# sontung/pyrenderer

Hardware: AMD Instinct MI355X
Metric: Msamples/sec Cornell box 512²×64spp at 1/2/4/8 GPU; per-pixel L2 vs CPU (higher is better)
Workload: dtype f32; 1 GPU; Cornell box (Lambertian) 512x512, 64 spp, depth 8; triangles=36, spheres=0, global_batch=16777216, parallelism=tiles1, collective=False, tile_scheme=latin, frames_in_flight=1, frames_per_launch=16, tile=64, bvh_depth=8, bvh_nodes=18

## Files before the change

### pyrenderer_amd/csrc/prt_capi.cpp

```cpp
#include <dlfcn.h>
#include <hip/hip_runtime.h>
#include <rccl/rccl.h>

#include <algorithm>
#include <cmath>
#include <cstdlib>
#include <cstring>
#include <map>
#include <memory>
#include <mutex>
#include <new>
#include <string>
#include <vector>

#include "../../include/prt.h"
#include "prt_internal.h"
#include "prt_kernels.h"

namespace {

thread_local std::string g_err;

int fail(int code, const std::string& msg) {
    g_err = msg;
// ... 3 lines not shown
#define HIP_TRY(expr)                                                                         \
    do {                                                                                      \
        hipError_t e_ = (expr);                                                               \
        if (e_ != hipSuccess) return fail(PRT_ERR_HIP, std::string(#expr) + ": " + hipGetErrorString(e_)); \
    } while (0)

float bits_f(int32_t v) { float f; std::memcpy(&f, &v, 4); return f; }

struct F3 { float x, y, z; };
F3 f3_norm(F3 a) {
    float l = std::sqrt(a.x * a.x + a.y * a.y + a.z * a.z);
    return F3{a.x / l, a.y / l, a.z / l};
}
F3 f3_cross(F3 a, F3 b) { return F3{a.y * b.z - a.z * b.y, a.z * b.x - a.x * b.z, a.x * b.y - a.y * b.x}; }
void frame_rows(F3 n, float* out12) {
    F3 v = f3_norm(n);
    F3 r1, r2, r3;
    if (v.y == 1.0f) {
        r1 = F3{1, 0, 0}; r2 = F3{0, 0, 1}; r3 = F3{0, 1, 0};
    } else if (v.y == -1.0f) {
        r1 = F3{1, 0, 0}; r2 = F3{0, 0, 1}; r3 = F3{0, -1, 0};
    } else {
        F3 x = f3_norm(f3_cross(v, F3{0.0f, 1.0f, 0.0f}));
        F3 z = f3_norm(f3_cross(x, v));
        r1 = x; r2 = z; r3 = v;
    }
    const F3 rows[3] = {r1, r2, r3};
    for (int k = 0; k < 3; ++k) {
        out12[4 * k] = rows[k].x; out12[4 * k + 1] = rows[k].y; out12[4 * k + 2] = rows[k].z; out12[4 * k + 3] = 0.0f;
    }
}

constexpr int kStatWords = 192;

struct DevBuf {
    void* p = nullptr;
    size_t bytes = 0;
    DevBuf() = default;
    DevBuf(const DevBuf&) = delete;
    DevBuf& operator=(const DevBuf&) = delete;
    ~DevBuf() { release(); }
    hipError_t ensure(size_t want) {
        if (want <= bytes) return hipSuccess;
        if (p) (void)hipFree(p);
        p = nullptr; bytes = 0;
        hipError_t e = hipMalloc(&p, want);
        if (e == hipSuccess) bytes = want;
        return e;
    }
    void release() { if (p) (void)hipFree(p); p = nullptr; bytes = 0; }
};

struct RenderCtx {
    hipStream_t stream = nullptr;
    DevBuf tiles, buf, rays, rays_o, work, acc, spill;
    std::vector<uint32_t> tile_host;
    uint64_t last_use = 0;
};
constexpr size_t kMaxCtx = 8;

struct Scene {
    int device = 0;
    int64_t n_tri = 0;
    int64_t n_nodes = 0;
    int32_t depth = 0;
    int n_light = 0;
    int n_mat = 0;
    int cus = 0;
    int blocks_per_cu = 0;
    int occ[2 * (prt::kVarLast + 1)] = {0};
    int n_lt = 0;
    int64_t n_tri_f4 = 0;
    float direct_rgb[3] = {0.9f, 0.85f, 0.7f};
    DevBuf nodes4q;
    int64_t n_node4q_f4 = 0;
    DevBuf nodes4, tris, tri_nm, tri_frame, mats, light_v, light_off, sph, sph_mat;
    int64_t n_node4_f4 = 0;
    int32_t depth4 = 0;
    int stack4 = 0;
    int need4 = 0;
    int leaf_break = -1;
    int leaf_exit = -1;
    int resume_min = 32;
    uint32_t guard_trips = 1u << 20;
    int spill_lds = 16;
    std::string wave_clock_path;
    int64_t n_sph = 0;
    bool plain = false;
    bool shade_fast = false;
    DevBuf work, stats;
    hipStream_t stream = nullptr;
    std::vector<std::unique_ptr<RenderCtx>> ctx;
    uint64_t use_clock = 0;
    std::vector<hipEvent_t> ev;
    int ev_used = 0;
    size_t chunk_bytes = (size_t)16 << 30;
    size_t device_bytes = 0;
    DevBuf frame, gather, gather_xy;
    std::vector<uint32_t> gather_xy_host;
    DevBuf scatter_xy;
    std::vector<uint32_t> scatter_xy_host;
    hipEvent_t scatter_ev = nullptr;
};

struct DeviceGuard {
    int prev = -1;
    explicit DeviceGuard(int dev) { (void)hipGetDevice(&prev); (void)hipSetDevice(dev); }
    ~DeviceGuard() { if (prev >= 0) (void)hipSetDevice(prev); }
};

int upload(DevBuf& b, const void* host, size_t bytes, size_t* total) {
    HIP_TRY(b.ensure(std::max<size_t>(bytes, 16)));
    if (bytes) HIP_TRY(hipMemcpy(b.p, host, bytes, hipMemcpyHostToDevice));
    *total += b.bytes;
    return PRT_OK;
}

void destroy_scene(Scene* s) {
    if (!s) return;
    DeviceGuard g(s->device);
    for (DevBuf* b : {&s->nodes4q, &s->nodes4, &s->tris, &s->tri_nm, &s->tri_frame, &s->mats, &s->light_v,
                      &s->light_off, &s->sph, &s->sph_mat, &s->work, &s->stats, &s->frame, &s->gather,
                      &s->gather_xy, &s->scatter_xy})
        b->release();
    if (!s->ctx.empty()) (void)hipDeviceSynchronize();
    for (auto& c : s->ctx)
        for (DevBuf* b : {&c->tiles, &c->buf, &c->rays, &c->rays_o, &c->work, &c->acc, &c->spill})
            b->release();
    for (hipEvent_t e : s->ev) (void)hipEventDestroy(e);
    if (s->scatter_ev) (void)hipEventDestroy(s->scatter_ev);
    if (s->stream) (void)hipStreamDestroy(s->stream);
    delete s;
}

int check_render_args(Scene* s, const float* cam, int W, int H, int tw, int th, const int32_t* tile_ids,
                      int n_tiles, int spp, int depth) {
    if (!s) return fail(PRT_ERR_ARG, "scene is NULL");
    if (!cam) return fail(PRT_ERR_ARG, "cam is NULL");
    if (W < 2 || H < 2) return fail(PRT_ERR_ARG, "W and H must be >= 2 (u = (x + r) / (W - 1))");
    if (tw < 1 || th < 1 || (tw & (tw - 1)) || (th & (th - 1)) || (int64_t)tw * th < 64 || (int64_t)tw * th > (1 << 20))
        return fail(PRT_ERR_ARG, "tile width/height must be powers of two with 64 <= tw*th <= 2^20");
    if (W > 65535 || H > 65535) return fail(PRT_ERR_ARG, "frame larger than 65535 pixels per side");
    if (n_tiles < 0 || (n_tiles > 0 && !tile_ids)) return fail(PRT_ERR_ARG, "bad tile list");
    if (spp < 0 || depth < 0) return fail(PRT_ERR_ARG, "spp and depth must be >= 0");
    int tiles_x = (W + tw - 1) / tw, tiles_y = (H + th - 1) / th;
    for (int i = 0; i < n_tiles; ++i)
        if (tile_ids[i] < 0 || tile_ids[i] >= tiles_x * tiles_y)
            return fail(PRT_ERR_ARG, "tile id out of range: " + std::to_string(tile_ids[i]));
    if ((int64_t)n_tiles * tw * th >= ((int64_t)1 << 31)) return fail(PRT_ERR_ARG, "too many pixels in one call");
    return PRT_OK;
}

constexpr size_t kFaultOffset = 32;

int take_fault_at(const DevBuf& work) {
    int f = 0;
    if (!work.p) return 0;
    if (hipMemcpy(&f, (char*)work.p + kFaultOffset, sizeof(int), hipMemcpyDeviceToHost) != hipSuccess) return -1;
    if (f != 0 && hipMemset((char*)work.p + kFaultOffset, 0, sizeof(int)) != hipSuccess) return -1;
    return f;
}
int take_fault(Scene* s) { return take_fault_at(s->work); }
int take_render_faults(Scene* s) {
    int any = 0;
    for (auto& c : s->ctx)
        if (int f = take_fault_at(c->work)) any = any ? any : f;
    return any;
}

RenderCtx* ctx_for(Scene* s, hipStream_t stream) {
    ++s->use_clock;
    for (auto& c : s->ctx)
        if (c->stream == stream) { c->last_use = s->use_clock; return c.get(); }
    if (s->ctx.size() >= kMaxCtx) {
        auto it = std::min_element(s->ctx.begin(), s->ctx.end(),
                                   [](const std::unique_ptr<RenderCtx>& a, const std::unique_ptr<RenderCtx>& b) {
                                       return a->last_use < b->last_use;
                                   });
        if (hipDeviceSynchronize() != hipSuccess) return nullptr;
        (*it)->stream = stream;
        (*it)->last_use = s->use_clock;
        return it->get();
    }
    auto c = std::unique_ptr<RenderCtx>(new (std::nothrow) RenderCtx());
    if (!c) return nullptr;
    if (c->work.ensure(64) != hipSuccess) return nullptr;
    if (hipMemset(c->work.p, 0, 64) != hipSuccess) return nullptr;
    c->stream = stream;
    c->last_use = s->use_clock;
    s->ctx.push_back(std::move(c));
    return s->ctx.back().get();
}

constexpr int64_t kLdsSceneBytes = 24 * 1024;
void scene_sizes(const Scene* s, prt::TraceParams& P) {
    P.n_node_f4 = (int)s->n_node4_f4;
    P.n_tri_f4 = (int)s->n_tri_f4;
    P.n_tri = (int)s->n_tri;
    P.n_mat = s->n_mat;
    P.n_lt = s->n_lt;
    P.n_light = s->n_light;
}
bool lds_fits4(const Scene* s) {
    prt::TraceParams P;
    std::memset(&P, 0, sizeof(P));
    scene_sizes(s, P);
    const int64_t n_refs = s->n_tri_f4 / 3;
    return (int64_t)prt::lds_scene_bytes(P) <= kLdsSceneBytes && s->n_node4_f4 / 8 < 0x7FFF && n_refs * 8 <= 32768;
}
int default_variant(const Scene* s, int64_t n_items = INT64_MAX) {
    (void)n_items;
    if (!lds_fits4(s) || !s->stack4) return prt::kVarGlobal;
    prt::TraceParams P;
    std::memset(&P, 0, sizeof(P));
    scene_sizes(s, P);
    P.lds_stack = s->need4;
    if (s->need4 <= 32 && prt::trace_smem_bytes(16, prt::kVarLdsPool, P) * 7 <= 160 * 1024)
        return prt::kVarLdsPool;
    size_t smem = prt::trace_smem_bytes(s->stack4, prt::kVarLds, P);
    return smem * 7 <= 160 * 1024 ? prt::kVarLds : smem * 6 <= 160 * 1024 ? prt::kVarLds6 : prt::kVarLdsAnyOcc;
}
int variant_stack(const Scene* s, int var) {
    return prt::variant_pool(var) ? 16 : prt::variant_spills(var) ? s->spill_lds : s->stack4;
}

bool camera_is_fast(const float* cam) {
    bool fin = true;
    for (int i = 0; i < 20; ++i) fin = fin && std::isfinite(cam[i]);
    return fin && !(cam[19] > 0.0f) && cam[12] == 0.0f && cam[13] == 0.0f && cam[14] == 0.0f && cam[15] == 1.0f;
}

void scene_params(Scene* s, prt::TraceParams& P) {
    std::memset(&P, 0, sizeof(P));
    P.nodes = (const float4*)s->nodes4.p;
    P.tris = (const float4*)s->tris.p;
    P.tri_nm = (const float4*)s->tri_nm.p;
    P.tri_frame = (const float4*)s->tri_frame.p;
    P.mats = (const float*)s->mats.p;
    P.light_v = (const float4*)s->light_v.p;
    P.light_off = (const int*)s->light_off.p;
    P.n_light = s->n_light;
    P.dl_r = s->direct_rgb[0]; P.dl_g = s->direct_rgb[1]; P.dl_b = s->direct_rgb[2];
    P.resume_min = s->resume_min;
    P.stats = (unsigned long long*)s->stats.p;
    scene_sizes(s, P);
    P.guard_trips = s->guard_trips;
    P.n_sph = (int)s->n_sph;
    P.sph = (const float4*)s->sph.p;
    P.sph_mat = (const int*)s->sph_mat.p;
    P.plain = s->plain ? 1 : 0;
    P.shade_fast = s->shade_fast ? 1 : 0;
    P.frame_spp = 0xFFFFFFFFu;
}

int launch_variant(const Scene* s, uint32_t flags, int64_t n_items) {
    int var = (int)((flags >> PRT_FLAG_VARIANT_SHIFT) & 0xFFu);
    const bool mis = (flags & PRT_FLAG_MIS_NEE) != 0;
    if (var == 0)
        var = !mis ? default_variant(s, n_items) : (lds_fits4(s) && s->stack4) ? prt::kVarLdsMis : prt::kVarGlobalMis;
    return var;
}

int trace_setup(Scene* s, RenderCtx* cx, uint32_t flags, int64_t n_items, prt::TraceParams& P, int* var_out,
                int* stack_out, int* occ_out) {
    const bool stats = (flags & PRT_FLAG_STATS) != 0;
    const bool mis = (flags & PRT_FLAG_MIS_NEE) != 0;
    int var = launch_variant(s, flags, n_items);
    if (var < prt::kVarFirst || var > prt::kVarLast) return fail(PRT_ERR_ARG, "unknown kernel variant");
    if (prt::variant_mis(var) != mis)
        return fail(PRT_ERR_ARG, "PRT_FLAG_MIS_NEE must be set exactly for the MIS estimator variants");
    const bool spill = prt::variant_spills(var);
    if (s->stack4 == 0 && !spill) return fail(PRT_ERR_ARG, "BVH4 too deep for the LDS traversal stack variants");
    const int stack = variant_stack(s, var);
    if (prt::variant_quantized(var)) {
        P.nodes = (const float4*)s->nodes4q.p;
        P.n_node_f4 = (int)s->n_node4q_f4;
    }
    if (prt::variant_uses_lds(var) && !lds_fits4(s)) return fail(PRT_ERR_ARG, "scene too large for the LDS variant");
    if (prt::variant_pool(var) && (s->need4 > 32 || s->need4 < 1))
        return fail(PRT_ERR_ARG, "BVH4 too deep for the pooled-shadow variant's LDS stack");
    const bool lds_var = prt::variant_uses_lds(var);
    P.lds_stack = s->need4;
    P.leaf_break = s->leaf_break >= 0 ? s->leaf_break : (lds_var ? 0 : 16);
    P.leaf_exit = s->leaf_exit >= 0 ? s->leaf_exit : (lds_var ? 8 : 24);
    int& occ = s->occ[2 * var + (stats ? 1 : 0)];
    if (occ == 0) occ = std::max(1, prt::trace_blocks_per_cu(stack, var, stats, prt::trace_smem_bytes(stack, var, P)));
    if (spill) {
        size_t per_lane = (size_t)std::max(1, s->need4 + 2 - s->spill_lds);
        HIP_TRY(cx->spill.ensure(per_lane * (size_t)occ * s->cus * 256 * sizeof(int)));
        P.spill = (int*)cx->spill.p;
    }
    *var_out = var;
    *stack_out = stack;
    *occ_out = occ;
    return PRT_OK;
}

void camera_params(prt::TraceParams& P, const float* cam, int W, int H, int tw, int th) {
    std::memcpy(P.cam, cam, sizeof(float) * PRT_CAM_FLOATS);
    P.cam_fast = camera_is_fast(cam) ? 1 : 0;
    const float rd2 = -cam[18];
    for (int i = 0; i < 3; ++i) {
        const float* c = cam + 4 * i;
        P.cam_o[i] = 0.0f * c[0] + 0.0f * c[1] + 0.0f * c[2] + 1.0f * c[3];
        P.cam_k[i] = rd2 * c[2];
    }
    P.W = W; P.H = H;
    P.wm1 = (float)(W - 1); P.hm1 = (float)(H - 1);
    P.log_tw = __builtin_ctz((unsigned)tw);
    P.log_tpx = __builtin_ctz((unsigned)(tw * th));
}

int enqueue_render(Scene* s, RenderCtx* cx, const float* cam, int W, int H, int tw, int th, const int32_t* tile_ids,
                   int n_tiles, int spp, int depth, uint64_t seed, uint32_t flags, float* d_acc,
                   int first_sample = 0, bool accumulate = false, int n_frames = 1, int frame_stride = 0,
                   int64_t out_pitch = 0) {
    if (flags & PRT_FLAG_NO_PRIMARY_KERNEL)
        return fail(PRT_ERR_UNSUP, "PRT_FLAG_NO_PRIMARY_KERNEL: camera rays always come from the camera kernel "
                                   "(the trace kernels no longer carry camera code)");
    const int64_t n_slots = (int64_t)n_tiles * tw * th;
    if (n_slots == 0) return PRT_OK;
    if (out_pitch == 0) out_pitch = 3 * n_slots;
    hipStream_t stream = cx->stream;
    const int tiles_x = (W + tw - 1) / tw;
    std::vector<uint32_t> origins((size_t)n_tiles);
    for (int i = 0; i < n_tiles; ++i)
        origins[(size_t)i] = ((uint32_t)((tile_ids[i] % tiles_x) * tw) << 16) | (uint32_t)((tile_ids[i] / tiles_x) * th);
    if (origins != cx->tile_host) {
        HIP_TRY(cx->tiles.ensure(sizeof(uint32_t) * (size_t)n_tiles));
        HIP_TRY(hipMemcpyAsync(cx->tiles.p, origins.data(), sizeof(uint32_t) * (size_t)n_tiles, hipMemcpyHostToDevice,
                               stream));
        cx->tile_host.swap(origins);
    }
    if (spp == 0 || depth == 0) {
        if (!accumulate)
            HIP_TRY(hipMemset2DAsync(d_acc, sizeof(float) * (size_t)out_pitch, 0, sizeof(float) * 3 * (size_t)n_slots,
                                     (size_t)n_frames, stream));
        return PRT_OK;
    }
    const int64_t T = (int64_t)spp * n_frames;
    const bool cam_fast = camera_is_fast(cam);
    int64_t per_sample = n_slots * 3 * (int64_t)sizeof(float);
    int64_t per_sample_all = per_sample + n_slots * (cam_fast ? 16 : 32);
    size_t budget = s->chunk_bytes;
    {
        const size_t held = cx->buf.bytes + cx->rays.bytes + cx->rays_o.bytes;
        size_t free_b = 0, total_b = 0;
        if ((size_t)(std::min<int64_t>(T, (int64_t)(budget / (size_t)per_sample_all)) * per_sample_all) > held &&
            hipMemGetInfo(&free_b, &total_b) == hipSuccess && free_b > 0)
            budget = std::min(budget, std::max<size_t>((size_t)per_sample_all, (free_b + held) / 2));
    }
    int64_t chunk = std::max<int64_t>(1, std::min<int64_t>(T, (int64_t)budget / per_sample_all));
    chunk = std::min<int64_t>(chunk, std::max<int64_t>(1, ((int64_t)1 << 31) / n_slots - 1));
    {
        const int64_t nc = (T + chunk - 1) / chunk;
        chunk = (T + nc - 1) / nc;
    }
    HIP_TRY(cx->buf.ensure((size_t)(chunk * per_sample)));
    HIP_TRY(cx->rays.ensure((size_t)(chunk * n_slots * 16)));
    if (!cam_fast) HIP_TRY(cx->rays_o.ensure((size_t)(chunk * n_slots * 16)));
    const bool stats = (flags & PRT_FLAG_STATS) != 0;
    const bool timed = (flags & PRT_FLAG_TIME) != 0;
    if (stats) HIP_TRY(hipMemsetAsync(s->stats.p, 0, kStatWords * sizeof(unsigned long long), stream));

    prt::TraceParams P;
    scene_params(s, P);
    camera_params(P, cam, W, H, tw, th);
    P.rays = (const float4*)cx->rays.p;
    P.ray_o = cam_fast ? nullptr : (const float4*)cx->rays_o.p;
// ... 216 lines not shown
    s->n_light = n_light;
    s->n_mat = n_mat;
    if (direct_rgb) std::memcpy(s->direct_rgb, direct_rgb, sizeof(float) * 3);
    DeviceGuard g(device);
    int rc = PRT_OK;
    do {
        hipError_t e = hipStreamCreateWithFlags(&s->stream, hipStreamNonBlocking);
        if (e != hipSuccess) { rc = fail(PRT_ERR_HIP, std::string("hipStreamCreate: ") + hipGetErrorString(e)); break; }
        std::vector<float> nm((size_t)std::max<int64_t>(n_tri, 1) * 4, 0.0f);
        for (int64_t i = 0; i < n_tri; ++i) {
            nm[4 * i] = tri_n[3 * i]; nm[4 * i + 1] = tri_n[3 * i + 1]; nm[4 * i + 2] = tri_n[3 * i + 2];
            nm[4 * i + 3] = bits_f(tri_mat[i]);
        }
        std::vector<float> fr((size_t)std::max<int64_t>(n_tri, 1) * 24, 0.0f);
        for (int64_t i = 0; i < n_tri; ++i) {
            F3 nn{tri_n[3 * i], tri_n[3 * i + 1], tri_n[3 * i + 2]};
            frame_rows(nn, fr.data() + 24 * i);
            frame_rows(F3{-nn.x, -nn.y, -nn.z}, fr.data() + 24 * i + 12);
        }
        int n_lt = light_off[n_light];
        s->n_lt = n_lt;
        std::vector<float> lv((size_t)n_lt * 16, 0.0f);
        for (int k = 0; k < n_lt; ++k) {
            int64_t t = light_tri[k];
            for (int c = 0; c < 3; ++c) {
                lv[16 * k + c] = tri_v[9 * t + c];
                lv[16 * k + 4 + c] = tri_v[9 * t + 3 + c];
                lv[16 * k + 8 + c] = tri_v[9 * t + 6 + c];
                lv[16 * k + 12 + c] = tri_n[3 * t + c];
            }
            lv[16 * k + 15] = bits_f(tri_mat[t]);
        }
        {
            prt::Bvh4Host b4;
            prt::collapse_bvh4(bvh, &b4);
            s->depth4 = b4.depth;
            s->n_node4_f4 = (int64_t)b4.nodes.size() / 4;
            s->stack4 = b4.stack_need <= 32 ? prt::stack_variant(b4.stack_need - 1) : 0;
            s->need4 = b4.stack_need;
            if ((rc = upload(s->nodes4, b4.nodes.data(), sizeof(float) * b4.nodes.size(), &s->device_bytes))) break;
            std::vector<float> q4;
            prt::quantize_bvh4(b4, bvh.pad, &q4);
            s->n_node4q_f4 = (int64_t)q4.size() / 4;
            if ((rc = upload(s->nodes4q, q4.data(), sizeof(float) * q4.size(), &s->device_bytes))) break;
        }
        if ((rc = upload(s->tris, bvh.tris.data(), sizeof(float) * bvh.tris.size(), &s->device_bytes))) break;
        if ((rc = upload(s->tri_nm, nm.data(), sizeof(float) * nm.size(), &s->device_bytes))) break;
        if ((rc = upload(s->tri_frame, fr.data(), sizeof(float) * fr.size(), &s->device_bytes))) break;
        if ((rc = upload(s->mats, mat, sizeof(float) * 8 * (size_t)n_mat, &s->device_bytes))) break;
        if ((rc = upload(s->light_v, lv.data(), sizeof(float) * lv.size(), &s->device_bytes))) break;
        if ((rc = upload(s->light_off, light_off, sizeof(int32_t) * (size_t)(n_light + 1), &s->device_bytes))) break;
        s->n_sph = n_sph;
        s->plain = n_sph == 0;
        for (int32_t i = 0; i < n_mat; ++i)
            if (mat[8 * i + 5] == 2.0f || mat[8 * i + 5] == 3.0f) s->plain = false;
        s->shade_fast = true;
        for (int32_t i = 0; i < n_mat && s->shade_fast; ++i)
            for (int c = 0; c < 3; ++c) {
                const float r = mat[8 * i + c];
                if (!(r >= 0x1p-40f && r <= 0x1p40f)) s->shade_fast = false;
            }
        for (int64_t i = 0; i < n_tri && s->shade_fast; ++i) {
            const double x = tri_n[3 * i], y = tri_n[3 * i + 1], z = tri_n[3 * i + 2];
            const double l2 = x * x + y * y + z * z;
            if (!(l2 >= 0.25 && l2 <= 4.0)) s->shade_fast = false;
        }
        if ((rc = upload(s->sph, sph, sizeof(float) * 4 * (size_t)n_sph, &s->device_bytes))) break;
        if ((rc = upload(s->sph_mat, sph_mat, sizeof(int32_t) * (size_t)n_sph, &s->device_bytes))) break;
        if ((e = s->work.ensure(64)) != hipSuccess || (e = s->stats.ensure(8 * kStatWords)) != hipSuccess) {
            rc = fail(PRT_ERR_OOM, std::string("hipMalloc: ") + hipGetErrorString(e));
            break;
        }
        if ((e = hipMemset(s->work.p, 0, 64)) != hipSuccess) { rc = fail(PRT_ERR_HIP, hipGetErrorString(e)); break; }
        hipDeviceProp_t prop;
        if ((e = hipGetDeviceProperties(&prop, device)) != hipSuccess) { rc = fail(PRT_ERR_HIP, hipGetErrorString(e)); break; }
        s->cus = prop.multiProcessorCount;
        s->n_tri_f4 = (int64_t)bvh.tris.size() / 4;
        if (const char* le = std::getenv("PRT_LEAF_EXIT")) s->leaf_exit = std::max(0, std::min(64, std::atoi(le)));
        if (const char* lb = std::getenv("PRT_LEAF_BREAK")) s->leaf_break = std::max(0, std::min(64, std::atoi(lb)));
        if (const char* wc = std::getenv("PRT_WAVE_CLOCK")) s->wave_clock_path = wc;
        if (const char* gt = std::getenv("PRT_GUARD_TRIPS"))
            s->guard_trips = (uint32_t)std::max(1LL, std::min((long long)UINT32_MAX, std::atoll(gt)));
        if (const char* rm = std::getenv("PRT_RESUME_MIN")) s->resume_min = std::max(1, std::min(64, std::atoi(rm)));
        if (const char* sl = std::getenv("PRT_SPILL_LDS")) {
            int v = std::atoi(sl);
            s->spill_lds = v == 4 ? 4 : v == 32 ? 32 : 16;
        }
        {
            prt::TraceParams Q;
            std::memset(&Q, 0, sizeof(Q));
            int var = default_variant(s);
            scene_sizes(s, Q);
            Q.lds_stack = s->need4;
            int stk = variant_stack(s, var);
            s->blocks_per_cu = std::max(1, prt::trace_blocks_per_cu(stk, var, false, prt::trace_smem_bytes(stk, var, Q)));
        }
        if (const char* cb = std::getenv("PRT_CHUNK_BYTES")) {
            s->chunk_bytes = (size_t)std::max(1LL << 20, std::atoll(cb));
        } else {
            size_t free_b = 0, total_b = 0;
            if (hipMemGetInfo(&free_b, &total_b) == hipSuccess && free_b > 0)
                s->chunk_bytes = std::max<size_t>((size_t)1 << 28, std::min(s->chunk_bytes, free_b / 4));
        }
    } while (0);
    if (rc != PRT_OK) { destroy_scene(s); return rc; }
    *out_scene = s;
    return PRT_OK;
}

int prt_scene_info(void* scene, int64_t* info8) {
    auto* s = (Scene*)scene;
    if (!s || !info8) return fail(PRT_ERR_ARG, "NULL argument");
    info8[0] = s->device; info8[1] = s->n_tri; info8[2] = s->n_nodes; info8[3] = s->depth;
    info8[4] = s->stack4; info8[5] = (int64_t)s->device_bytes; info8[6] = s->blocks_per_cu; info8[7] = s->cus;
    return PRT_OK;
}

int prt_closest_hits(void* scene, const float* rays, int64_t n, uint32_t flags, int32_t* hit_id, float* hit_t) {
    auto* s = (Scene*)scene;
    if (!s || (n > 0 && (!rays || !hit_id || !hit_t))) return fail(PRT_ERR_ARG, "NULL argument");
    if (n < 0) return fail(PRT_ERR_ARG, "n < 0");
    if (n == 0) return PRT_OK;
    if (s->need4 > 64) return fail(PRT_ERR_ARG, "BVH4 too deep for the hit-query kernel");
    DeviceGuard g(s->device);
    const bool quant = (flags & PRT_HITS_QUANTIZED) != 0, any = (flags & PRT_HITS_ANY) != 0;
    prt::TraceParams P;
    std::memset(&P, 0, sizeof(P));
    P.nodes = (const float4*)(quant ? s->nodes4q.p : s->nodes4.p);
    P.tris = (const float4*)s->tris.p;
    P.n_tri = (int)s->n_tri;
    P.n_sph = (int)s->n_sph;
    P.sph = (const float4*)s->sph.p;
    DevBuf d_rays, d_id, d_t;
    HIP_TRY(d_rays.ensure(sizeof(float) * 8 * (size_t)n));
    HIP_TRY(d_id.ensure(sizeof(int32_t) * (size_t)n));
    HIP_TRY(d_t.ensure(sizeof(float) * (size_t)n));
    P.fault = (int*)((char*)s->work.p + kFaultOffset);
    P.guard_trips = s->guard_trips;
    HIP_TRY(hipMemsetAsync(P.fault, 0, sizeof(int), s->stream));
    HIP_TRY(hipMemcpyAsync(d_rays.p, rays, sizeof(float) * 8 * (size_t)n, hipMemcpyHostToDevice, s->stream));
    HIP_TRY(prt::launch_hits(P, quant, any, 64, (const float4*)d_rays.p, n, (int*)d_id.p, (float*)d_t.p, s->stream));
    HIP_TRY(hipMemcpyAsync(hit_id, d_id.p, sizeof(int32_t) * (size_t)n, hipMemcpyDeviceToHost, s->stream));
    HIP_TRY(hipMemcpyAsync(hit_t, d_t.p, sizeof(float) * (size_t)n, hipMemcpyDeviceToHost, s->stream));
    HIP_TRY(hipStreamSynchronize(s->stream));
    if (take_fault(s) != 0) return fail(PRT_ERR_INTERNAL, "traversal watchdog tripped (corrupt acceleration structure?)");
    return PRT_OK;
}

int prt_hit_all(void* scene, const float* rays, int64_t n, uint64_t seed, uint32_t flags, float* out16) {
    auto* s = (Scene*)scene;
    if (!s || (n > 0 && (!rays || !out16))) return fail(PRT_ERR_ARG, "NULL argument");
    if (n < 0) return fail(PRT_ERR_ARG, "n < 0");
    if (flags & ~PRT_HITS_QUANTIZED) return fail(PRT_ERR_ARG, "prt_hit_all takes only PRT_HITS_QUANTIZED");
    if (n == 0) return PRT_OK;
    if (s->need4 > 64) return fail(PRT_ERR_ARG, "BVH4 too deep for the hit-query kernel");
    DeviceGuard g(s->device);
    const bool quant = (flags & PRT_HITS_QUANTIZED) != 0;
    prt::TraceParams P;
    scene_params(s, P);
    if (quant) P.nodes = (const float4*)s->nodes4q.p;
    P.seed_lo = (uint32_t)seed; P.seed_hi = (uint32_t)(seed >> 32);
    P.fault = (int*)((char*)s->work.p + kFaultOffset);
    DevBuf d_rays, d_id, d_t, d_out;
    HIP_TRY(d_rays.ensure(sizeof(float) * 8 * (size_t)n));
    HIP_TRY(d_id.ensure(sizeof(int32_t) * (size_t)n));
    HIP_TRY(d_t.ensure(sizeof(float) * (size_t)n));
// ... 543 lines not shown
```

### pyrenderer_amd/csrc/prt_device.h

```cpp
#pragma once
#pragma clang fp contract(off)

#include <hip/hip_runtime.h>
#include <type_traits>
#include <stdint.h>

#include "prt_kernels.h"

namespace prt {
namespace {

constexpr float kInvPi = 0.31830988618379067154f;
constexpr float kPiOver4 = 0.78539816339744830961f;
constexpr float kTMin = 0.00001f;
constexpr float kTMax = 99999.9f;
constexpr float kGamma = 0x1.000006p+0f;
constexpr int kBlock = 256;
constexpr int kChunk = 64;

struct V3 { float x, y, z; };
__device__ __forceinline__ V3 v3(float x, float y, float z) { return V3{x, y, z}; }
__device__ __forceinline__ V3 operator+(V3 a, V3 b) { return v3(a.x + b.x, a.y + b.y, a.z + b.z); }
__device__ __forceinline__ V3 operator-(V3 a, V3 b) { return v3(a.x - b.x, a.y - b.y, a.z - b.z); }
__device__ __forceinline__ V3 operator*(V3 a, V3 b) { return v3(a.x * b.x, a.y * b.y, a.z * b.z); }
// ... 1225 lines not shown
        const float4* src = nodes + 8 * n;
        float4 v = slot == 6 ? src[6] : src[2 * ax + (sgn ^ far)];
        if (slot == 6) {
            int* rr = reinterpret_cast<int*>(&v);
            for (int c = 0; c < 4; ++c) rr[c] = rr[c] == kSentinel ? LdsStack16::kSent : rr[c];
        }
        float key[4];
        {
            const float4 lx = src[0], hx = src[1], ly = src[2], hy = src[3], lz = src[4], hz = src[5];
            const float4 rf = src[6];
            const int rr[4] = {__float_as_int(rf.x), __float_as_int(rf.y), __float_as_int(rf.z), __float_as_int(rf.w)};
            const float nxv[4] = {lx.x, lx.y, lx.z, lx.w}, fxv[4] = {hx.x, hx.y, hx.z, hx.w};
            const float nyv[4] = {ly.x, ly.y, ly.z, ly.w}, fyv[4] = {hy.x, hy.y, hy.z, hy.w};
            const float nzv[4] = {lz.x, lz.y, lz.z, lz.w}, fzv[4] = {hz.x, hz.y, hz.z, hz.w};
            for (int c = 0; c < 4; ++c) {
                key[c] = rr[c] == kSentinel ? INFINITY
                                            : ((k & 1) ? -fxv[c] : nxv[c]) + ((k & 2) ? -fyv[c] : nyv[c]) +
                                                  ((k & 4) ? -fzv[c] : nzv[c]);
                if (!(key[c] == key[c])) key[c] = INFINITY;
            }
        }
        const float vin[4] = {v.x, v.y, v.z, v.w};
        int rank[4];
#pragma unroll
        for (int c = 0; c < 4; ++c) {
            rank[c] = 0;
#pragma unroll
            for (int e = 0; e < 4; ++e) rank[c] += (key[e] < key[c] || (key[e] == key[c] && e < c)) ? 1 : 0;
        }
        float vout[4];
#pragma unroll
        for (int j = 0; j < 4; ++j)
            vout[j] = rank[0] == j ? vin[0] : rank[1] == j ? vin[1] : rank[2] == j ? vin[2] : vin[3];
        sn[i] = make_float4(vout[0], vout[1], vout[2], vout[3]);
    }
}

constexpr int kPoolF4 = 7 * kBlock / 4;
constexpr int kQueueF4 = 2 * kBlock / 16;
constexpr int kCtlF4 = 3;
#ifndef PRT_POOL_S_PRIO
#define PRT_POOL_S_PRIO 2
#endif

template <bool STATS, int WPE, bool PLAIN>
__global__ __attribute__((amdgpu_flat_work_group_size(kBlock, kBlock), amdgpu_waves_per_eu(WPE)))
void trace_kernel_pool(TraceParams P) {
    constexpr int ctl_f4 = kCtlF4;
    extern __shared__ float4 smem[];
    const int tid = threadIdx.x;
    const int lane = tid & 63;
    const int stack_f4 = P.lds_stack * kBlock * 2 / 16;
    LdsStack16A stk;
    stk.base = (int)(uintptr_t)(LdsShort*)(reinterpret_cast<short*>(smem) + (tid & ~63) + 2 * (tid & 31) +
                                           ((tid >> 5) & 1));
    using Stk = decltype(stk);
    float* pool = reinterpret_cast<float*>(smem + stack_f4);
    uint8_t* queue = reinterpret_cast<uint8_t*>(smem + stack_f4 + kPoolF4);
    uint32_t* ctl = reinterpret_cast<uint32_t*>(smem + stack_f4 + kPoolF4 + kQueueF4);
    float4* sn = smem + stack_f4 + kPoolF4 + kQueueF4 + ctl_f4;
    const int n_node4 = P.n_node_f4 / 8;
    float4* st4 = sn + 56 * n_node4;
    float4* slv = st4 + P.n_tri_f4;
    int* slo = reinterpret_cast<int*>(slv + 4 * P.n_lt);
    float4* smt = slv + 4 * P.n_lt + (P.n_light + 4) / 4;
    copy_octant_nodes(sn, P.nodes, n_node4);
    for (int i = tid; i < P.n_tri_f4; i += kBlock) st4[i] = P.tris[i];
    for (int i = tid; i < 4 * P.n_lt; i += kBlock) slv[i] = P.light_v[i];
    for (int i = tid; i <= P.n_light; i += kBlock) slo[i] = P.light_off[i];
    for (int i = tid; i < 2 * P.n_mat; i += kBlock) smt[i] = reinterpret_cast<const float4*>(P.mats)[i];
    if (tid < 4 * ctl_f4) ctl[tid] = 0u;
    __syncthreads();
    const float4* g_nodes = sn;
    const float4* g_tris = st4;
    const float4* s_nm = P.tri_nm;
    const float4* s_fr = P.tri_frame;
    const float* s_mats = reinterpret_cast<const float*>(smt);

    uint32_t q_next = 0, q_end = 0;
    bool exhausted = false;
    int item = -1;
    int bounce = 0;
    bool my_sh = false;
    uint32_t st = 0;
    V3 o = v3(0, 0, 0), d = v3(0, 0, 0), wi = v3(0, 0, 0);
    V3 beta = v3(1, 1, 1), L = v3(0, 0, 0), pend = v3(0, 0, 0);
    Counters cn = {0, 0, 0, 0, 0, 0, 0, 0, 0, 0, 0, 0, 0, 0, 0};
    uint64_t n_e = 0, n_s = 0, lanes_s = 0, pre_hits = 0;
    uint64_t lt[16] = {0, 0, 0, 0, 0, 0, 0, 0, 0, 0, 0, 0, 0, 0, 0, 0};
    auto book_trav = [&](int k) {
        lt[k] += cn.wi; lt[k + 1] += cn.li; lt[k + 2] += cn.wl; lt[k + 3] += cn.ll;
        cn.wi = 0; cn.li = 0; cn.wl = 0; cn.ll = 0;
    };
    auto book = [&](int k) {
        uint32_t w = 0, l = 0;
        wave_tick(w, l);
        lt[k] += w; lt[k + 1] += l;
    };
    uint32_t chunk_s = 0, chunk_xy0 = 0;
    uint32_t slot = 0, slot_prev = 0, nch_prev = 0;
    uint32_t qpar = 0;
#ifdef PRT_POOL_CLOCKS
    uint64_t ck[6] = {0, 0, 0, 0, 0, 0};
    uint64_t t_c = __builtin_amdgcn_s_memtime();
#define PRT_CLOCK(k) do { const uint64_t t_n = __builtin_amdgcn_s_memtime(); ck[k] += t_n - t_c; t_c = t_n; } while (0)
#else
#define PRT_CLOCK(k) do {} while (0)
#endif
    auto refill = [&](KParams& Q) {
            bool me_idle = item < 0;
            uint64_t idle = __ballot(me_idle);
            for (int round = 0; round < 2 && idle; ++round) {
                uint32_t avail = q_end - q_next;
                if (avail == 0 && !exhausted) {
                    uint32_t base = 0;
                    if (lane == 0) base = atomicAdd(Q.work, (uint32_t)kChunk);
                    base = __builtin_amdgcn_readfirstlane(base);
                    if ((uint64_t)base >= Q.n_items) {
                        exhausted = true;
                    } else {
                        q_next = base;
                        q_end = (uint32_t)min((uint64_t)base + kChunk, Q.n_items);
                        chunk_s = __builtin_amdgcn_readfirstlane(base / (uint32_t)Q.n_slots);
                        uint32_t tk = (base - chunk_s * (uint32_t)Q.n_slots) >> Q.log_tpx;
                        chunk_xy0 = ((const __attribute__((address_space(4))) uint32_t*)(uintptr_t)Q.tile_xy)[tk];
                    }
                    avail = q_end - q_next;
                }
                if (avail == 0) break;
                uint32_t rank = __builtin_amdgcn_mbcnt_hi((uint32_t)(idle >> 32), __builtin_amdgcn_mbcnt_lo((uint32_t)idle, 0u));
                uint32_t need = (uint32_t)__popcll(idle);
                uint32_t take = need < avail ? need : avail;
                if (me_idle && rank < take) {
                    item = (int)(q_next + rank);
                    L = v3(0, 0, 0);
                    int x, y;
                    pixel_of(Q, (uint32_t)item, chunk_s, chunk_xy0, x, y);
                    int W = Q.W, H = Q.H;
                    asm volatile("" : "+s"(W), "+s"(H));
                    bool ok = x < W && y < H;
                    if (ok) {
                        float4 r = Q.rays[item];
                        d = v3(r.x, r.y, r.z);
                        st = __float_as_uint(r.w);
                        if (Q.ray_o) {
                            const float4 ro = Q.ray_o[item];
                            o = v3(ro.x, ro.y, ro.z);
                        } else {
                            float o0 = Q.cam_o[0], o1 = Q.cam_o[1], o2 = Q.cam_o[2];
                            asm volatile("" : "+s"(o0), "+s"(o1), "+s"(o2));
                            o = v3(o0, o1, o2);
                        }
                    }
                    if (!ok) {
                        float* out = Q.out + (size_t)item * 3;
                        out[0] = 0.0f; out[1] = 0.0f; out[2] = 0.0f;
                        item = -2;
                    } else {
                        beta = v3(1, 1, 1);
                        bounce = 0;
                        pool[0 * kBlock + tid] = o.x; pool[1 * kBlock + tid] = o.y; pool[2 * kBlock + tid] = o.z;
                        wi = d;
                    }
                }
                q_next += take;
                me_idle = item == -1;
                idle = __ballot(me_idle);
            }
        if (item == -2) item = -1;
    };
    while (true) {
        KParams& Q = kernarg();
        refill(Q);
        PRT_CLOCK(4);
        if (STATS && item >= 0) book(12);
        const bool trav = item >= 0 && !(my_sh && bounce + 1 >= Q.depth);
        int hid = -1;
        float ht = 0.0f;
        bool hit = false;
        if (__ballot(trav) != 0) {
            if (STATS && lane == __builtin_amdgcn_readfirstlane(lane)) n_e++;
            if (trav) {
                if (STATS) { cn.ext++; cn.q0 = cn.nodes; }
                hit = traverse_ww4<STATS, 1, Stk, false, false, true>(
                    g_nodes, g_tris, o, d, kTMin, kTMax, false, stk, hid, ht, cn, nullptr, 0, Q.fault,
                    exhausted ? 0 : Q.leaf_break, exhausted ? 0 : Q.leaf_exit, Q.guard_trips);
                if (STATS) { cn.max_q = max(cn.max_q, cn.nodes - cn.q0); book_trav(0); }
                if (!PLAIN && Q.n_sph > 0) {
                    float best = hit ? ht : kTMax;
                    for (int k = 0; k < Q.n_sph; ++k) {
                        float root;
                        if (sphere_hit(Q.sph[k], o, d, kTMin, best, root)) {
                            best = root;
                            hid = Q.n_tri + k;
                            hit = true;
                        }
                    }
                    ht = best;
                }
            }
        }
        PRT_CLOCK(5);
        if (__ballot(my_sh) != 0) {
            bool late = false;
            const uint32_t need = nch_prev;
            for (uint32_t spin = 0;
                 need && __hip_atomic_load(&ctl[9 + slot_prev], __ATOMIC_ACQUIRE, __HIP_MEMORY_SCOPE_WORKGROUP) < need;
                 ++spin) {
                if (spin >= (1u << 20)) {
                    if (lane == 0) atomicOr(Q.fault, 2);
                    late = true;
                    break;
                }
                __builtin_amdgcn_s_sleep(1);
            }
            if (my_sh) {
                if (STATS) book(14);
                const float r = pool[6 * kBlock + tid];
                if (late) L = v3(__int_as_float(0x7FC00000), __int_as_float(0x7FC00000), __int_as_float(0x7FC00000));
                else if (r == r) L = L + pend;
                my_sh = false;
                ++bounce;
                if (bounce >= Q.depth) {
                    float* out = Q.out + (size_t)item * 3;
                    out[0] = L.x; out[1] = L.y; out[2] = L.z;
                    if (STATS && !(isfinite(L.x) && isfinite(L.y) && isfinite(L.z))) cn.nonfinite++;
                    item = -1;
                }
            }
        }
        if (trav) {
            if (STATS) book(8);
            {
                bool finished = false;
                if (!hit) {
                    finished = true;
                } else {
                    V3 p = o + d * ht;
                    V3 ng;
                    int mid;
                    if (PLAIN || hid < Q.n_tri) {
                        float4 nm = s_nm[hid];
                        ng = xyz(nm);
                        mid = __float_as_int(nm.w);
                    } else {
                        asm volatile("");
                        float4 sc = Q.sph[hid - Q.n_tri];
                        ng = v3((p.x - sc.x) / sc.w, (p.y - sc.y) / sc.w, (p.z - sc.z) / sc.w);
                        mid = Q.sph_mat[hid - Q.n_tri];
                    }
                    const float* m = s_mats + 8 * mid;
                    const bool flip = m[4] == 0.0f && dot(ng, neg(d)) < 0.0f;
                    const V3 n = flip ? neg(ng) : ng;
                    if (!PLAIN && (m[5] == 2.0f || m[5] == 3.0f)) {
                        bool front = dot(d, ng) < 0.0f;
                        V3 ns = front ? ng : neg(ng);
                        V3 unit = normalize(d);
                        V3 out;
                        bool absorbed = false;
                        if (m[5] == 2.0f) {
                            out = reflect3(unit, ns);
                            if (m[7] > 0.0f) out = out + random_in_unit_sphere(st) * m[7];
                            absorbed = !(dot(out, ns) > 0.0f);
                        } else {
                            float ratio = front ? 1.0f / m[6] : m[6];
                            float ct = -dot(unit, ns);
                            ct = ct > 1.0f ? 1.0f : ct;
                            float stn = sqrtf(1.0f - ct * ct);
                            bool cannot = ratio * stn > 1.0f;
                            if (cannot || schlick(ct, ratio) > rng_next(st)) out = reflect3(unit, ns);
                            else out = refract3(unit, ns, ratio);
                        }
                        if (absorbed) {
                            finished = true;
                        } else {
                            beta = beta * v3(m[0], m[1], m[2]);
                            wi = normalize(out);
                            ++bounce;
                            if (bounce >= Q.depth) finished = true;
                        }
                    } else if (m[3] != 0.0f) {
                        float d1 = dot(neg(d), n);
                        if (d1 > 0.0f) {
                            V3 lc = v3(Q.dl_r, Q.dl_g, Q.dl_b);
                            L = bounce == 0 ? L + lc * beta : L + (lc * beta) * d1;
                        }
                        finished = true;
                    } else {
                        if (STATS) book(10);
                        float u0 = rng_next(st);
                        float u1 = rng_next(st);
                        V3 l = cosine_hemisphere<true>(u0, u1);
                        const float4* fr = s_fr + ((size_t)((PLAIN || hid < Q.n_tri) ? hid : 0) * 2 + (flip ? 1 : 0)) * 3;
                        if (PLAIN || hid < Q.n_tri) {
                            float4 f0 = fr[0], f1 = fr[1], f2 = fr[2];
                            wi = normalize<true>(xyz(f0) * l.x + xyz(f1) * l.y + xyz(f2) * l.z);
                        } else {
                            wi = to_world(n, l);
                        }
                        float pdf = fabsf(dot(n, wi)) * kInvPi;
                        V3 att = v3(m[0], m[1], m[2]);
                        float cw = dot(n, wi);
                        float dz = cw > 0.0f ? cw : 0.0f;
                        V3 ad = v3(att.x * dz, att.y * dz, att.z * dz);
                        V3 adp = lambert_div<true>(ad, pdf, cw, Q.shade_fast);
                        V3 nb = v3(adp.x * kInvPi, adp.y * kInvPi, adp.z * kInvPi);
                        beta = beta * nb;
                        int li = Q.n_light > 1 ? rng_int(st, 0, Q.n_light - 1) : 0;
                        int lo = slo[li];
                        int f = rng_int(st, 0, slo[li + 1] - lo - 1);
                        float su = sqrt_cr<true>(rng_next(st));
                        float sv = rng_next(st);
                        float a = su * (1.0f - sv);
                        float b = su * sv;
                        const float4* lv = slv + (size_t)(lo + f) * 4;
                        float4 L0 = lv[0], L1 = lv[1], L2 = lv[2], LN = lv[3];
                        float c = 1.0f - a - b;
                        V3 p2 = (xyz(L0) * a + xyz(L1) * b) + xyz(L2) * c;
                        V3 n2 = xyz(LN);
                        V3 w = normalize<true>(p2 - p);
                        float t_at = (p2.x - p.x) / w.x;
                        float dot1 = dot(n, w), dot2 = -dot(n2, w);
                        bool queued = false;
                        if (dot1 > 0.0f && dot2 > 0.0f) {
                            if (STATS) cn.shadow++;
                            float tl;
                            const V3 lv0 = xyz(L0);
                            const bool self_hit = mt_u(lv0, xyz(L1) - lv0, xyz(L2) - lv0, p, w, kTMin, t_at, 0, -1,
                                                       true, tl);
                            if (STATS) { cn.tris++; pre_hits += self_hit ? 1 : 0; }
                            if (!self_hit) {
                                const float* em = s_mats + 8 * __float_as_int(LN.w);
                                V3 dd = p - p2;
                                float sl = dot(dd, dd);
                                V3 rad = nee_div<true>(v3(em[0] * dot1 * dot2, em[1] * dot1 * dot2, em[2] * dot1 * dot2), sl,
                                                         dot1, dot2, Q.shade_fast);
                                pend = beta * rad;
                                pool[3 * kBlock + tid] = w.x; pool[4 * kBlock + tid] = w.y; pool[5 * kBlock + tid] = w.z;
                                pool[6 * kBlock + tid] = t_at;
                                queued = true;
                            }
                        }
                        if (queued) {
                            my_sh = true;
                        } else {
                            ++bounce;
                            if (bounce >= Q.depth) finished = true;
                        }
                    }
                    pool[0 * kBlock + tid] = p.x; pool[1 * kBlock + tid] = p.y; pool[2 * kBlock + tid] = p.z;
                }
                if (finished) {
                    float* out = Q.out + (size_t)item * 3;
                    out[0] = L.x; out[1] = L.y; out[2] = L.z;
                    if (STATS && !(isfinite(L.x) && isfinite(L.y) && isfinite(L.z))) cn.nonfinite++;
                    item = -1;
                }
            }
        }
        {
            const uint64_t m = __ballot(my_sh);
            const uint32_t cnt = (uint32_t)__popcll(m);
            uint32_t base = 0;
            if (cnt) {
                if (lane == __builtin_amdgcn_readfirstlane(lane)) base = atomicAdd(&ctl[slot], cnt);
                base = __builtin_amdgcn_readfirstlane(base);
                const uint32_t rank = __builtin_amdgcn_mbcnt_hi((uint32_t)(m >> 32), __builtin_amdgcn_mbcnt_lo((uint32_t)m, 0u));
                if (my_sh) queue[qpar * kBlock + base + rank] = (uint8_t)tid;
            }
            if ((__ballot(item >= 0) != 0 || !exhausted) && lane == 0) ctl[3 + slot] = 1u;
            if (tid == 0) {
                const uint32_t ns = slot == 2 ? 0u : slot + 1u;
                ctl[ns] = 0u; ctl[3 + ns] = 0u; ctl[6 + ns] = 0u; ctl[9 + ns] = 0u;
            }
        }
        PRT_CLOCK(0);
        __syncthreads();
        PRT_CLOCK(1);
        const uint32_t n_q = ctl[slot];
        const uint32_t n_chunks = (n_q + 63u) >> 6;
        uint32_t chunk = 0xFFFFFFFFu;
        if (n_chunks) {
            if (lane == 0) chunk = atomicAdd(&ctl[6 + slot], 1u);
            chunk = __builtin_amdgcn_readfirstlane(chunk);
        }
        if (chunk < n_chunks) {
            __builtin_amdgcn_s_setprio(PRT_POOL_S_PRIO);
            const uint32_t e0 = chunk * 64u, e1 = min(n_q, e0 + 64u);
            const uint32_t e = e0 + (uint32_t)lane;
            if (STATS && lane == 0) { n_s++; lanes_s += e1 - e0; }
            const bool sq = e < e1;
            int owner = 0;
            V3 so = v3(0, 0, 0), sd = v3(1, 1, 1);
            float stm = 0.0f;
            if (sq) {
                owner = queue[qpar * kBlock + e];
                so = v3(pool[0 * kBlock + owner], pool[1 * kBlock + owner], pool[2 * kBlock + owner]);
                sd = v3(pool[3 * kBlock + owner], pool[4 * kBlock + owner], pool[5 * kBlock + owner]);
                stm = pool[6 * kBlock + owner];
            }
            if (sq) {
                int hid = -1;
                float ht = 0.0f;
                if (STATS) cn.q0 = cn.nodes;
                bool hit = traverse_ww4<STATS, 2, Stk, false, false, true>(
                    g_nodes, g_tris, so, sd, kTMin, stm, true, stk, hid, ht, cn, nullptr, 0, Q.fault,
                    exhausted ? 0 : Q.leaf_break, exhausted ? 0 : Q.leaf_exit, Q.guard_trips);
                if (STATS) { cn.max_q = max(cn.max_q, cn.nodes - cn.q0); book_trav(4); }
                if (!PLAIN && Q.n_sph > 0 && !hit) {
                    for (int k = 0; k < Q.n_sph; ++k) {
                        float root;
                        if (sphere_hit(Q.sph[k], so, sd, kTMin, stm, root)) { hit = true; break; }
                    }
                }
                pool[6 * kBlock + owner] = hit ? __int_as_float(0x7FC00000) : 0.0f;
            }
            __builtin_amdgcn_s_setprio(0);
            __builtin_amdgcn_fence(__ATOMIC_RELEASE, "workgroup");
            if (lane == 0) __hip_atomic_fetch_add(&ctl[9 + slot], 1u, __ATOMIC_RELEASE, __HIP_MEMORY_SCOPE_WORKGROUP);
        }
        nch_prev = n_chunks;
        PRT_CLOCK(2);
        const bool alive = ctl[3 + slot] != 0u;
        slot_prev = slot;
        slot = slot == 2 ? 0u : slot + 1u;
        qpar ^= 1u;
        o = v3(pool[0 * kBlock + tid], pool[1 * kBlock + tid], pool[2 * kBlock + tid]);
        d = wi;
        if (!alive) break;
    }
#ifdef PRT_POOL_CLOCKS
    if (lane == 0)
        for (int k = 0; k < 6; ++k) atomicAdd(P.stats + 24 + k, (unsigned long long)ck[k]);
#endif
#undef PRT_CLOCK
    if (STATS) {
        uint64_t a = cn.nodes, b = cn.tris, c = cn.ext, e = cn.shadow;
        for (int off = 32; off > 0; off >>= 1) {
            a += __shfl_down(a, off); b += __shfl_down(b, off);
            c += __shfl_down(c, off); e += __shfl_down(e, off);
        }
        uint64_t ph[5] = {n_e, n_s, lanes_s, pre_hits, 0};
        for (int k = 0; k < 4; ++k)
            for (int off = 32; off > 0; off >>= 1) ph[k] += __shfl_down(ph[k], off);
        if (lane == 0) {
            atomicAdd(P.stats + 0, (unsigned long long)a);
            atomicAdd(P.stats + 1, (unsigned long long)b);
            atomicAdd(P.stats + 2, (unsigned long long)c);
            atomicAdd(P.stats + 3, (unsigned long long)e);
            for (int k = 0; k < 4; ++k) atomicAdd(P.stats + 17 + k, (unsigned long long)ph[k]);
        }
        for (int k = 0; k < 16; ++k) {
            uint64_t v = lt[k];
            for (int off = 32; off > 0; off >>= 1) v += __shfl_down(v, off);
            if (lane == 0 && v) atomicAdd(P.stats + 160 + k, (unsigned long long)v);
        }
        uint32_t msp = cn.max_sp, nf = cn.nonfinite, mq = cn.max_q;
        for (int off = 32; off > 0; off >>= 1) {
            msp = max(msp, (uint32_t)__shfl_down((int)msp, off));
            nf += (uint32_t)__shfl_down((int)nf, off);
            mq = max(mq, (uint32_t)__shfl_down((int)mq, off));
        }
        if (lane == 0) {
            atomicMax(P.stats + 13, (unsigned long long)msp);
            if (nf) atomicAdd(P.stats + 14, (unsigned long long)nf);
            atomicMax(P.stats + 16, (unsigned long long)mq);
        }
    }
}

}

#define PRT_VARIANTS(X)                       \
    X(kVarLds, 8, true, 7)                    \
    X(kVarLdsAnyOcc, 8, true, 1)              \
    X(kVarGlobal, 224, false, 6)              \
    X(kVarLdsMis, 256, true, 6)               \
    X(kVarLds6, 8, true, 6)                   \
    X(kVarGlobalMis, 480, false, 6)           \
    X(kVarLdsPool, 512, true, 7)              \
    X(kVarLdsPool6, 512, true, 6)

template <int STACK, bool STATS, int VAR, bool LDS, int WPE>
static hipError_t launch_one(const TraceParams& P, int grid, size_t smem, hipStream_t stream) {
    constexpr bool spill = (VAR & 32) != 0;
    if constexpr ((VAR & 512) != 0) {
        if constexpr (STACK == 16) return launch_trace_pool(P, STATS, WPE, grid, smem, stream);
        else return hipErrorInvalidValue;
    } else if constexpr (spill ? (STACK == 4 || STACK == 16 || STACK == 32) : (STACK != 4)) {
        trace_kernel<STACK, STATS, VAR, LDS, WPE><<<grid, kBlock, smem, stream>>>(P);
        return hipGetLastError();
    } else {
        return hipErrorInvalidValue;
    }
}

template <int STACK, bool STATS>
static hipError_t launch_var(const TraceParams& P, int var, int grid, size_t smem, hipStream_t stream) {
    switch (var) {
#define X(id, bits, lds, wpe) \
        case id: return launch_one<STACK, STATS, bits, lds, wpe>(P, grid, smem, stream);
        PRT_VARIANTS(X)
#undef X
        default: return hipErrorInvalidValue;
    }
}

template <int STACK, bool STATS, int VAR, bool LDS, int WPE>
static void occ_one(int* n, size_t smem) {
    constexpr bool spill = (VAR & 32) != 0;
    if constexpr ((VAR & 512) != 0) {
        if constexpr (STACK == 16) *n = trace_occ_pool(STATS, WPE, smem);
    } else if constexpr (spill ? (STACK == 4 || STACK == 16 || STACK == 32) : (STACK != 4))
        (void)hipOccupancyMaxActiveBlocksPerMultiprocessor(n, trace_kernel<STACK, STATS, VAR, LDS, WPE>, kBlock, smem);
}

template <int STACK, bool STATS>
static int occ_var(int var, size_t smem) {
    int n = 0;
    switch (var) {
#define X(id, bits, lds, wpe) \
        case id: occ_one<STACK, STATS, bits, lds, wpe>(&n, smem); break;
        PRT_VARIANTS(X)
#undef X
        default: break;
    }
    return n;
}

}
```

### pyrenderer_amd/csrc/prt_kernels.h

```cpp
#pragma once
#include <hip/hip_runtime.h>
#include <stdint.h>

namespace prt {

struct TraceParams {
    const float4* nodes;
    const float4* tris;
    const float4* tri_nm;
    const float4* tri_frame;
    const float* mats;
    const float4* light_v;
    const int* light_off;
    int n_light;
    float dl_r, dl_g, dl_b;
    float cam[24];
    int cam_fast;
    int* fault;
    uint32_t guard_trips;
    int leaf_break;
    int leaf_exit;
    int resume_min;
    int* spill;
    const float4* rays;
    const float4* ray_o;
    float cam_o[3], cam_k[3];
    int W, H;
    float wm1, hm1;
    int log_tw, log_tpx;
    const uint32_t* tile_xy;
    int n_slots;
    int s0;
    uint32_t j0, frame_spp, frame_stride;
    int depth;
    uint32_t seed_lo, seed_hi;
    uint64_t n_items;
    uint32_t* work;
    float* out;
    unsigned long long* stats;
    int n_node_f4, n_tri_f4;
    int n_mat, n_lt;
    int n_tri;
    int n_sph;
    const float4* sph;
    const int* sph_mat;
    unsigned long long* wave_clock;
    int cam_clears;
    int lds_stack;
    int plain;
    int shade_fast;
};

constexpr int kVarLds = 1;
constexpr int kVarLdsAnyOcc = 2;
constexpr int kVarGlobal = 3;
constexpr int kVarLdsMis = 4;
constexpr int kVarGlobalMis = 5;
constexpr int kVarLds6 = 6;
constexpr int kVarLdsPool = 7;
constexpr int kVarLdsPool6 = 8;
constexpr int kVarFirst = 1;
constexpr int kVarLast = 8;
bool variant_pool(int var);
bool variant_mis(int var);
bool variant_uses_lds(int var);
bool variant_spills(int var);
bool variant_quantized(int var);

int stack_variant(int bvh_depth);
size_t trace_smem_bytes(int stack, int var, const TraceParams& P);
hipError_t launch_camera(const TraceParams& P, float4* rays, float4* ray_o, hipStream_t stream);
hipError_t launch_hits(const TraceParams& P, bool quantized, bool any, int stack, const float4* rays, int64_t n,
                       int* hit_id, float* hit_t, hipStream_t stream);
hipError_t launch_hit_shade(const TraceParams& P, const float4* rays, int64_t n, const int* hit_id, const float* hit_t,
                            float* out16, hipStream_t stream);
hipError_t launch_rays_prep(const TraceParams& P, const float* in8, int64_t n, int64_t n_pad, float4* rays,
                            float4* ray_o, hipStream_t stream);
size_t lds_scene_bytes(const TraceParams& P);
hipError_t launch_trace(const TraceParams& P, int stack, int var, int grid, bool stats, hipStream_t stream);
hipError_t launch_reduce(const float* buf, float* acc, int n_slots, int64_t j0, int64_t n, int64_t spp, int64_t f0,
                         int64_t n_frames, int64_t pitch, bool accumulate, hipStream_t stream);
hipError_t launch_scatter(const float* packed, const uint32_t* tile_xy, int n_slots, int log_tw, int log_tpx, int x0,
                          int y0, int w, int h, float* out, hipStream_t stream);
hipError_t launch_scatter_frames(const float* packed, const uint32_t* tile_xy, int n_slots, int group_slots,
                                 int64_t group_pitch, int n_frames, int64_t src_fpitch, int64_t dst_fpitch, int log_tw,
                                 int log_tpx, int x0, int y0, int w, int h, float* out, hipStream_t stream);
int trace_blocks_per_cu(int stack, int var, bool stats, size_t smem);
hipError_t launch_rcp_selftest(unsigned long long* d_out, hipStream_t stream);
hipError_t launch_guard_selftest(unsigned long long* d_out, hipStream_t stream);
hipError_t launch_trace_pool(const TraceParams& P, bool stats, int wpe, int grid, size_t smem, hipStream_t stream);
int trace_occ_pool(bool stats, int wpe, size_t smem);

}
```

Baseline: 4605 Msamples/s.

## Suspend long pool-kernel traversals and let free lanes claim shadow rays individually

In the pooled-shadow trace kernel, extension-ray traversal can now suspend once fewer than a minimum number of lanes are still active. Its state (node, leaf, stack pointer, best hit) is saved in LDS and resumed on the next iteration. Shadow-queue work is no longer claimed in fixed 64-entry chunks: each wave claims as many entries as it has non-suspended lanes, and completion is counted per entry. The aim is to cut divergence stalls where a few long-traversing lanes hold up a whole wave, at the cost of extra LDS save/restore traffic and more complex queue accounting.

```diff
diff --git a/pyrenderer_amd/csrc/prt_capi.cpp b/pyrenderer_amd/csrc/prt_capi.cpp
--- a/pyrenderer_amd/csrc/prt_capi.cpp
+++ b/pyrenderer_amd/csrc/prt_capi.cpp
@@ -109,6 +109,7 @@
     int leaf_break = -1;
     int leaf_exit = -1;
     int resume_min = 32;
+    int pool_resume_min = 12;
     uint32_t guard_trips = 1u << 20;
     int spill_lds = 16;
     std::string wave_clock_path;
@@ -269,6 +270,7 @@
     P.n_light = s->n_light;
     P.dl_r = s->direct_rgb[0]; P.dl_g = s->direct_rgb[1]; P.dl_b = s->direct_rgb[2];
     P.resume_min = s->resume_min;
+    P.pool_resume_min = s->pool_resume_min;
     P.stats = (unsigned long long*)s->stats.p;
     scene_sizes(s, P);
     P.guard_trips = s->guard_trips;
@@ -312,6 +314,7 @@
     P.leaf_exit = s->leaf_exit >= 0 ? s->leaf_exit : (lds_var ? 8 : 24);
     int& occ = s->occ[2 * var + (stats ? 1 : 0)];
     if (occ == 0) occ = std::max(1, prt::trace_blocks_per_cu(stack, var, stats, prt::trace_smem_bytes(stack, var, P)));
+    if (n_items <= (int64_t)occ * s->cus * 256) P.pool_resume_min = 0;
     if (spill) {
         size_t per_lane = (size_t)std::max(1, s->need4 + 2 - s->spill_lds);
         HIP_TRY(cx->spill.ensure(per_lane * (size_t)occ * s->cus * 256 * sizeof(int)));
@@ -694,6 +697,7 @@
         if (const char* gt = std::getenv("PRT_GUARD_TRIPS"))
             s->guard_trips = (uint32_t)std::max(1LL, std::min((long long)UINT32_MAX, std::atoll(gt)));
         if (const char* rm = std::getenv("PRT_RESUME_MIN")) s->resume_min = std::max(1, std::min(64, std::atoi(rm)));
+        if (const char* pr = std::getenv("PRT_POOL_RESUME_MIN")) s->pool_resume_min = std::max(0, std::min(64, std::atoi(pr)));
         if (const char* sl = std::getenv("PRT_SPILL_LDS")) {
             int v = std::atoi(sl);
             s->spill_lds = v == 4 ? 4 : v == 32 ? 32 : 16;
diff --git a/pyrenderer_amd/csrc/prt_device.h b/pyrenderer_amd/csrc/prt_device.h
--- a/pyrenderer_amd/csrc/prt_device.h
+++ b/pyrenderer_amd/csrc/prt_device.h
@@ -1331,11 +1331,13 @@
     int item = -1;
     int bounce = 0;
     bool my_sh = false;
+    bool susp = false;
     uint32_t st = 0;
     V3 o = v3(0, 0, 0), d = v3(0, 0, 0), wi = v3(0, 0, 0);
     V3 beta = v3(1, 1, 1), L = v3(0, 0, 0), pend = v3(0, 0, 0);
     Counters cn = {0, 0, 0, 0, 0, 0, 0, 0, 0, 0, 0, 0, 0, 0, 0};
     uint64_t n_e = 0, n_s = 0, lanes_s = 0, pre_hits = 0;
+    uint64_t n_susp = 0, n_res = 0;
     uint64_t lt[16] = {0, 0, 0, 0, 0, 0, 0, 0, 0, 0, 0, 0, 0, 0, 0, 0};
     auto book_trav = [&](int k) {
         lt[k] += cn.wi; lt[k + 1] += cn.li; lt[k + 2] += cn.wl; lt[k + 3] += cn.ll;
@@ -1347,7 +1349,7 @@
         lt[k] += w; lt[k + 1] += l;
     };
     uint32_t chunk_s = 0, chunk_xy0 = 0;
-    uint32_t slot = 0, slot_prev = 0, nch_prev = 0;
+    uint32_t slot = 0, slot_prev = 0, nq_prev = 0;
     uint32_t qpar = 0;
 #ifdef PRT_POOL_CLOCKS
     uint64_t ck[6] = {0, 0, 0, 0, 0, 0};
@@ -1426,16 +1428,30 @@
         const bool trav = item >= 0 && !(my_sh && bounce + 1 >= Q.depth);
         int hid = -1;
         float ht = 0.0f;
-        bool hit = false;
+        bool hit = false, done = false;
+        TState ts = {0, 0, 0, 0, 0.0f};
         if (__ballot(trav) != 0) {
             if (STATS && lane == __builtin_amdgcn_readfirstlane(lane)) n_e++;
             if (trav) {
-                if (STATS) { cn.ext++; cn.q0 = cn.nodes; }
-                hit = traverse_ww4<STATS, 1, Stk, false, false, true>(
-                    g_nodes, g_tris, o, d, kTMin, kTMax, false, stk, hid, ht, cn, nullptr, 0, Q.fault,
-                    exhausted ? 0 : Q.leaf_break, exhausted ? 0 : Q.leaf_exit, Q.guard_trips);
-                if (STATS) { cn.max_q = max(cn.max_q, cn.nodes - cn.q0); book_trav(0); }
-                if (!PLAIN && Q.n_sph > 0) {
+                if (susp) {
+                    const uint32_t cl = __float_as_uint(pool[3 * kBlock + tid]), sb = __float_as_uint(pool[4 * kBlock + tid]);
+                    ts.cur = (int)(short)(cl & 0xFFFFu); ts.leaf = (int)cl >> 16;
+                    ts.sp = (int)(sb & 0xFFFFu); ts.best_id = (int)sb >> 16;
+                    ts.best = pool[5 * kBlock + tid];
+                    if (STATS) n_res++;
+                } else {
+                    tstate_init(ts, stk, kTMax);
+                    if (STATS) { cn.ext++; cn.q0 = cn.nodes; }
+                }
+                done = traverse_ww4<STATS, 1, Stk, false, true, true>(
+                    g_nodes, g_tris, o, d, kTMin, kTMax, false, stk, hid, ht, cn, &ts, exhausted ? 0 : Q.pool_resume_min + 1,
+                    Q.fault, exhausted ? 0 : Q.leaf_break, exhausted ? 0 : Q.leaf_exit, Q.guard_trips);
+                hit = done && hid >= 0;
+                if (STATS) {
+                    if (done) cn.max_q = max(cn.max_q, cn.nodes - cn.q0);
+                    book_trav(0);
+                }
+                if (!PLAIN && done && Q.n_sph > 0) {
                     float best = hit ? ht : kTMax;
                     for (int k = 0; k < Q.n_sph; ++k) {
                         float root;
@@ -1452,7 +1468,7 @@
         PRT_CLOCK(5);
         if (__ballot(my_sh) != 0) {
             bool late = false;
-            const uint32_t need = nch_prev;
+            const uint32_t need = nq_prev;
             for (uint32_t spin = 0;
                  need && __hip_atomic_load(&ctl[9 + slot_prev], __ATOMIC_ACQUIRE, __HIP_MEMORY_SCOPE_WORKGROUP) < need;
                  ++spin) {
@@ -1478,7 +1494,14 @@
                 }
             }
         }
-        if (trav) {
+        susp = trav && !done;
+        if (susp) {
+            pool[3 * kBlock + tid] = __uint_as_float(((uint32_t)ts.cur & 0xFFFFu) | ((uint32_t)ts.leaf << 16));
+            pool[4 * kBlock + tid] = __uint_as_float(((uint32_t)ts.sp & 0xFFFFu) | ((uint32_t)ts.best_id << 16));
+            pool[5 * kBlock + tid] = ts.best;
+            if (STATS) n_susp++;
+        }
+        if (trav && done) {
             if (STATS) book(8);
             {
                 bool finished = false;
@@ -1627,18 +1650,20 @@
         __syncthreads();
         PRT_CLOCK(1);
         const uint32_t n_q = ctl[slot];
-        const uint32_t n_chunks = (n_q + 63u) >> 6;
-        uint32_t chunk = 0xFFFFFFFFu;
-        if (n_chunks) {
-            if (lane == 0) chunk = atomicAdd(&ctl[6 + slot], 1u);
-            chunk = __builtin_amdgcn_readfirstlane(chunk);
-        }
-        if (chunk < n_chunks) {
+        const uint64_t free_m = __ballot(!susp);
+        const uint32_t n_free = (uint32_t)__popcll(free_m);
+        uint32_t e0 = 0xFFFFFFFFu;
+        if (n_q && n_free) {
+            if (lane == 0) e0 = atomicAdd(&ctl[6 + slot], n_free);
+            e0 = __builtin_amdgcn_readfirstlane(e0);
+        }
+        if (e0 < n_q) {
             __builtin_amdgcn_s_setprio(PRT_POOL_S_PRIO);
-            const uint32_t e0 = chunk * 64u, e1 = min(n_q, e0 + 64u);
-            const uint32_t e = e0 + (uint32_t)lane;
+            const uint32_t e1 = min(n_q, e0 + n_free);
+            const uint32_t e = e0 + __builtin_amdgcn_mbcnt_hi((uint32_t)(free_m >> 32),
+                                                             __builtin_amdgcn_mbcnt_lo((uint32_t)free_m, 0u));
             if (STATS && lane == 0) { n_s++; lanes_s += e1 - e0; }
-            const bool sq = e < e1;
+            const bool sq = !susp && e < e1;
             int owner = 0;
             V3 so = v3(0, 0, 0), sd = v3(1, 1, 1);
             float stm = 0.0f;
@@ -1666,9 +1691,9 @@
             }
             __builtin_amdgcn_s_setprio(0);
             __builtin_amdgcn_fence(__ATOMIC_RELEASE, "workgroup");
-            if (lane == 0) __hip_atomic_fetch_add(&ctl[9 + slot], 1u, __ATOMIC_RELEASE, __HIP_MEMORY_SCOPE_WORKGROUP);
-        }
-        nch_prev = n_chunks;
+            if (lane == 0) __hip_atomic_fetch_add(&ctl[9 + slot], e1 - e0, __ATOMIC_RELEASE, __HIP_MEMORY_SCOPE_WORKGROUP);
+        }
+        nq_prev = n_q;
         PRT_CLOCK(2);
         const bool alive = ctl[3 + slot] != 0u;
         slot_prev = slot;
@@ -1703,6 +1728,11 @@
             uint64_t v = lt[k];
             for (int off = 32; off > 0; off >>= 1) v += __shfl_down(v, off);
             if (lane == 0 && v) atomicAdd(P.stats + 160 + k, (unsigned long long)v);
+        }
+        for (int off = 32; off > 0; off >>= 1) { n_susp += __shfl_down(n_susp, off); n_res += __shfl_down(n_res, off); }
+        if (lane == 0 && n_susp) {
+            atomicAdd(P.stats + 176, (unsigned long long)n_susp);
+            atomicAdd(P.stats + 177, (unsigned long long)n_res);
         }
         uint32_t msp = cn.max_sp, nf = cn.nonfinite, mq = cn.max_q;
         for (int off = 32; off > 0; off >>= 1) {
diff --git a/pyrenderer_amd/csrc/prt_kernels.h b/pyrenderer_amd/csrc/prt_kernels.h
--- a/pyrenderer_amd/csrc/prt_kernels.h
+++ b/pyrenderer_amd/csrc/prt_kernels.h
@@ -49,6 +49,7 @@
     int lds_stack;
     int plain;
     int shade_fast;
+    int pool_resume_min;
 };
 
 constexpr int kVarLds = 1;
```

After: 4878 Msamples/s, median of 6. 5.9% higher.
